# JSzitas/nlsolver

Hardware: AMD Instinct MI355X
Metric: candidate-evals/sec (pop x iters/s) Rosenbrock-128D DE (higher is better)
Workload: dtype f64; 1 GPU; Rosenbrock-128D DE strategy=random CR=0.9 F=0.8, pop=65536 per GPU (BASELINE configs[1]), one step = best scan + std_err + stop tests + one generation; global_pop=65536, dim=128

## Files before the change

nlsolver_amd/csrc/nlsg_common.h:

```cpp
#pragma once

#ifdef __HIPCC_RTC__
typedef unsigned long long uint64_t;
typedef long long int64_t;
typedef unsigned int uint32_t;
typedef int int32_t;
typedef unsigned char uint8_t;
#else
#include <hip/hip_runtime.h>
#include <stdint.h>

#include <atomic>
#include <chrono>
#include <cstdarg>
#include <cstdio>
#include <cstring>
#endif

#include "../../include/nlsg_c_api.h"
#include "nlsg_math.h"
#ifndef __HIPCC_RTC__
#include "nlsg_pool.h"
#endif

// ... 137 lines not shown
  const uint32_t hi = lane_xor32<OFF>(static_cast<uint32_t>(v >> 32));
  return (static_cast<uint64_t>(hi) << 32) | lo;
}
template <int OFF>
__device__ inline double lane_xor(double v) {
  return __longlong_as_double(static_cast<long long>(
      lane_xor<OFF>(static_cast<uint64_t>(__double_as_longlong(v)))));
}
__device__ inline double lane_down1(double v) {
  const uint64_t b = static_cast<uint64_t>(__double_as_longlong(v));
  const uint32_t lo = dpp_mov32<0x130, 0xF>(static_cast<uint32_t>(b), static_cast<uint32_t>(b));
  const uint32_t hi = dpp_mov32<0x130, 0xF>(static_cast<uint32_t>(b >> 32), static_cast<uint32_t>(b >> 32));
  return __longlong_as_double(static_cast<long long>((static_cast<uint64_t>(hi) << 32) | lo));
}
__device__ inline double lane_up1(double v) {
  const uint64_t b = static_cast<uint64_t>(__double_as_longlong(v));
  const uint32_t lo = dpp_mov32<0x138, 0xF>(static_cast<uint32_t>(b), static_cast<uint32_t>(b));
  const uint32_t hi = dpp_mov32<0x138, 0xF>(static_cast<uint32_t>(b >> 32), static_cast<uint32_t>(b >> 32));
  return __longlong_as_double(static_cast<long long>((static_cast<uint64_t>(hi) << 32) | lo));
}
__device__ inline double lane_first(double v) {
  const uint64_t b = static_cast<uint64_t>(__double_as_longlong(v));
  const uint32_t lo = __builtin_amdgcn_readfirstlane(static_cast<int>(b & 0xffffffffu));
  const uint32_t hi = __builtin_amdgcn_readfirstlane(static_cast<int>(b >> 32));
  return __longlong_as_double(static_cast<long long>((static_cast<uint64_t>(hi) << 32) | lo));
}
__device__ inline double lane_last(double v) {
  const uint64_t b = static_cast<uint64_t>(__double_as_longlong(v));
  const uint32_t lo = __builtin_amdgcn_readlane(static_cast<int>(b & 0xffffffffu), 63);
  const uint32_t hi = __builtin_amdgcn_readlane(static_cast<int>(b >> 32), 63);
  return __longlong_as_double(static_cast<long long>((static_cast<uint64_t>(hi) << 32) | lo));
}
__device__ inline uint64_t on_valu(uint64_t s) {
  const uint32_t lo = static_cast<uint32_t>(s), hi = static_cast<uint32_t>(s >> 32);
  uint32_t vlo, vhi;
  asm("v_mov_b32 %0, %1" : "=v"(vlo) : "s"(lo));
  asm("v_mov_b32 %0, %1" : "=v"(vhi) : "s"(hi));
  return (static_cast<uint64_t>(vhi) << 32) | vlo;
}
__device__ inline uint64_t first64(uint64_t v) {
  const uint32_t lo = __builtin_amdgcn_readfirstlane(static_cast<int>(v & 0xffffffffu));
  const uint32_t hi = __builtin_amdgcn_readfirstlane(static_cast<int>(v >> 32));
  return (static_cast<uint64_t>(hi) << 32) | lo;
}
__device__ inline uint64_t readlane64(uint64_t v, int src) {
  const uint32_t lo = __builtin_amdgcn_readlane(static_cast<int>(v & 0xffffffffu), src);
  const uint32_t hi = __builtin_amdgcn_readlane(static_cast<int>(v >> 32), src);
  return (static_cast<uint64_t>(hi) << 32) | lo;
}
__device__ inline double lane_broadcast(double v, int src) {
  return __longlong_as_double(static_cast<long long>(
      readlane64(static_cast<uint64_t>(__double_as_longlong(v)), src)));
}
__device__ inline bool lane_bit(uint64_t m) {
#if __has_builtin(__builtin_amdgcn_inverse_ballot_w64)
  return __builtin_amdgcn_inverse_ballot_w64(m);
#else
  uint32_t r;
  asm("v_cndmask_b32_e64 %0, 0, 1, %1" : "=v"(r) : "s"(m));
  return r != 0;
#endif
}
template <int N>
struct int_c {
  static constexpr int value = N;
};
template <int FIRST, typename F>
__device__ inline void butterfly_levels(F &&f) {
  f(int_c<FIRST>{});
  if constexpr (FIRST > 1) butterfly_levels<FIRST / 2>(f);
}

template <int CTRL, int BANK>
__device__ inline uint32_t dpp_fresh32(uint32_t src) {
  return static_cast<uint32_t>(__builtin_amdgcn_mov_dpp(static_cast<int>(src), CTRL, 0xF, BANK, true));
}
template <int OFF>
__device__ inline double xor_add(double v) {
  static_assert(OFF == 1 || OFF == 2 || OFF == 4 || OFF == 8 || OFF == 16 || OFF == 32, "");
  const uint64_t b = static_cast<uint64_t>(__double_as_longlong(v));
  const uint32_t lo = static_cast<uint32_t>(b), hi = static_cast<uint32_t>(b >> 32);
  auto f64 = [](uint32_t l, uint32_t h) {
    return __longlong_as_double(static_cast<long long>((static_cast<uint64_t>(h) << 32) | l));
  };
  if constexpr (OFF == 16 || OFF == 32) {
    if constexpr (OFF == 16) {
      const auto rl = __builtin_amdgcn_permlane16_swap(lo, lo, false, false);
      const auto rh = __builtin_amdgcn_permlane16_swap(hi, hi, false, false);
      return f64(rl[0], rh[0]) + f64(rl[1], rh[1]);
    } else {
      const auto rl = __builtin_amdgcn_permlane32_swap(lo, lo, false, false);
      const auto rh = __builtin_amdgcn_permlane32_swap(hi, hi, false, false);
      return f64(rl[0], rh[0]) + f64(rl[1], rh[1]);
    }
  } else if constexpr (OFF == 4) {
    const uint32_t pl = dpp_mov32<0x114, 0xA>(dpp_fresh32<0x104, 0x5>(lo), lo);
    const uint32_t ph = dpp_mov32<0x114, 0xA>(dpp_fresh32<0x104, 0x5>(hi), hi);
    return v + f64(pl, ph);
  } else {
    constexpr int ctrl = OFF == 1 ? 0xB1 : OFF == 2 ? 0x4E : 0x128;
    return v + f64(dpp_fresh32<ctrl, 0xF>(lo), dpp_fresh32<ctrl, 0xF>(hi));
  }
}

__device__ inline double wave_sum(double v) {
  butterfly_levels<32>([&](auto off) { v = xor_add<decltype(off)::value>(v); });
// ... 640 lines not shown
```

nlsolver_amd/csrc/nlsg_de_kernels.h:

```cpp
#pragma once

#include "nlsg_common.h"
#include "nlsg_de_state.h"

namespace nlsg {

constexpr int kTraceWords = 5;

struct DeParams {
  double *buf[2];
  double *scores[2];
  uint8_t *home[2];
  double *best_x;
  uint64_t *trace;
  DeState *state;
  TilePartial *part;
  uint32_t *ticket;
  const double *zero;
  uint32_t ntiles;
  uint32_t stream;
  uint64_t pop, D, shard_lo, shard_n;
  double CR, F, eps, fmul;
  uint64_t max_iter, best_val_no_change, seed;
  int32_t strategy;
// ... 332 lines not shown
  const uint32_t d32 = static_cast<uint32_t>(D);
  auto row = [&](uint32_t h, uint64_t local) {
    return ((h & 1u) ? p.buf[1] : p.buf[0]) + static_cast<uint64_t>(static_cast<uint32_t>(local)) * d32;
  };
  auto load2 = [&](const double *rp, double (&v)[2]) {
    v[0] = in0 ? rp[j0] : 0.0;
    v[1] = in1 ? rp[j1] : 0.0;
  };
  double d1[2], d2[2], d3[2], keep[2];
  load2(row(hp[r0 - p.shard_lo], r0 - p.shard_lo), d1);
  load2(row(hp[r1 - p.shard_lo], r1 - p.shard_lo), d2);
  load2(row(hp[r2 - p.shard_lo], r2 - p.shard_lo), d3);
  const double *ks = rnd ? row(ha, a) : p.best_x;
  keep[0] = (in0 && !cross[0]) ? ks[j0] : 0.0;
  keep[1] = (in1 && !cross[1]) ? ks[j1] : 0.0;
  const double old_score = p.scores[par][a];
  double trial[2];
#pragma unroll
  for (int k = 0; k < 2; k++) {
    const double mut = d1[k] + p.F * (d2[k] - d3[k]);
    const double t = cross[k] ? mut : keep[k];
    trial[k] = (k ? in1 : in0) ? t : 0.0;
  }
  const double score = p.fmul * group_objective<OBJ, G>(trial[0], trial[1], D);
  const bool accept = score < old_score;
  if (live) {
    if (accept) {
      double *out = row(ha ^ 1u, a);
      if (in0) out[j0] = trial[0];
      if (in1) out[j1] = trial[1];
    }
    if (g == 0) {
      p.scores[par ^ 1][a] = accept ? score : old_score;
      p.home[par ^ 1][a] = static_cast<uint8_t>(accept ? ha ^ 1u : ha);
      if (p.trace != nullptr) {
        uint64_t *t = p.trace + a * kTraceWords;
        t[0] = r0;
        t[1] = r1;
        t[2] = r2;
        t[3] = jrand;
        t[4] = accept ? 1u : 0u;
      }
    }
  }
}

template <int OBJ, int G>
__global__ __launch_bounds__(256) void de_generation_groups_kernel(DeParams p, int par,
                                                                   uint64_t generation,
                                                                   int ignore_done) {
  de_generation_groups_block<OBJ, G>(p, par, generation, ignore_done, blockIdx.x);
}

template <int OBJ, bool VEC>
__device__ inline void de_generation_pair(const DeParams &p, int par, uint64_t generation, uint64_t block) {
  static_assert(TermsNonNegative<OBJ>::value, "the screen needs terms >= 0");
  using O = Objective<OBJ>;
  const uint64_t a0 = 2 * (block * 4 + __builtin_amdgcn_readfirstlane(static_cast<int>(threadIdx.x) >> 6));
  if (a0 >= p.shard_n) return;
  const bool two = a0 + 1 < p.shard_n;
  const int lane = lane_id();
  const uint32_t j = static_cast<uint32_t>(lane) & 31u;
  const bool upper = lane >= 32;
  const bool live = !upper || two;
  const uint32_t a = static_cast<uint32_t>(a0) + ((upper && two) ? 1u : 0u);
  const uint8_t *__restrict__ hp = p.home[par];
  const uint32_t hraw = hp[a];
  double old_score = p.scores[par][a];
  const uint32_t d32 = static_cast<uint32_t>(p.D);
  const uint64_t ka = ctr_key(p.gen_key, p.shard_lo + a);
  const uint32_t lim = j == 0 ? d32 : static_cast<uint32_t>(p.shard_n);
  const uint32_t idx = static_cast<uint32_t>(u01(mix64(ka + golden_times(d32 + j + 1u))) * static_cast<double>(lim));
  const uint32_t drawn = idx >= lim ? lim - 1 : idx;
  uint32_t sel = hraw;
  asm("" : "+v"(sel), "+v"(old_score) : "v"(drawn));
  const uint32_t cnt = (sel >> 2) & 3u;
  const bool tries = live & de_screen_tries(sel, generation, a, p.retry_mask, p.screen_retry_mask);
  bool dec = false;
  uint32_t left = cnt << 2;
  if (__ballot(tries) != 0ull) {
    const uint32_t hsel = hp[(j >= 1 && j < 8) ? drawn : a];
    auto half_of = [&](uint32_t lo, uint32_t hi) { return upper ? hi : lo; };
    auto lane32 = [&](uint32_t v, int src) {
      return static_cast<uint32_t>(__builtin_amdgcn_readlane(static_cast<int>(v), src));
    };
    const uint32_t jrand = half_of(lane32(drawn, 0), lane32(drawn, 32));
    constexpr uint32_t top = 1u << 31;
    const uint64_t b0 = __ballot(drawn != a) & ~0x0000000100000001ull;
    const uint32_t m0l = static_cast<uint32_t>(b0), m0h = static_cast<uint32_t>(b0 >> 32);
    const int i0l = __builtin_ctz(m0l | top), i0h = __builtin_ctz(m0h | top);
    const uint32_t r0 = half_of(lane32(drawn, i0l), lane32(drawn, 32 + i0h));
    const uint64_t b1 = __ballot(drawn != r0);
    const uint32_t m1l = m0l & static_cast<uint32_t>(b1) & ((~0u << i0l) << 1);
    const uint32_t m1h = m0h & static_cast<uint32_t>(b1 >> 32) & ((~0u << i0h) << 1);
    const int i1l = __builtin_ctz(m1l | top), i1h = __builtin_ctz(m1h | top);
    const uint32_t r1 = half_of(lane32(drawn, i1l), lane32(drawn, 32 + i1h));
    const uint64_t b2 = __ballot(drawn != r1);
    const uint32_t m2l = m1l & static_cast<uint32_t>(b2) & ((~0u << i1l) << 1);
    const uint32_t m2h = m1h & static_cast<uint32_t>(b2 >> 32) & ((~0u << i1h) << 1);
    const int i2l = __builtin_ctz(m2l | top), i2h = __builtin_ctz(m2h | top);
    const uint32_t r2 = half_of(lane32(drawn, i2l), lane32(drawn, 32 + i2h));
    const bool okl = m0l != 0 && m1l != 0 && m2l != 0 && i2l < 8;
    const bool okh = m0h != 0 && m1h != 0 && m2h != 0 && i2h < 8;
    const bool run = tries && (upper ? okh : okl);
    const uint32_t h0 = half_of(lane32(hsel, i0l), lane32(hsel, 32 + i0h));
    const uint32_t h1 = half_of(lane32(hsel, i1l), lane32(hsel, 32 + i1h));
    const uint32_t h2 = half_of(lane32(hsel, i2l), lane32(hsel, 32 + i2h));
    const uint64_t ka_lane = ka + golden_times(2 * j + 1u);
    const bool c0 = mix64(ka_lane) < p.cr_thresh || p.cr_all || 2 * j == jrand;
    const bool c1 = mix64(ka_lane + kGolden) < p.cr_thresh || p.cr_all || 2 * j + 1 == jrand;
    typedef double __attribute__((address_space(1))) global_double;
    global_double *base0 = (global_double *)p.buf[0], *base1 = (global_double *)p.buf[1];
    asm("" : "+s"(base0), "+s"(base1));
    auto load2 = [&](uint32_t h, uint32_t r, double (&v)[2]) {
      const double *src = (double *)((h & 1u) ? base1 : base0) + static_cast<uint64_t>(r) * d32 + 2 * j;
      if (VEC) {
        const double2 t = *reinterpret_cast<const double2 *>(src);
        v[0] = t.x;
        v[1] = t.y;
      } else {
        v[0] = src[0];
        v[1] = src[1];
      }
    };
    double d1[2], d2[2], d3[2];
    load2(h0, r0, d1);
    load2(h1, r1, d2);
    load2(h2, r2, d3);
    const double x0 = d1[0] + p.F * (d2[0] - d3[0]);
    const double x1 = d1[1] + p.F * (d2[1] - d3[1]);
    const double xn = lane_down1(x0);
    const bool cn = lane_bit(__ballot(c0) >> 1) && j != 31;
    const bool k0 = c0 && (O::kChain ? c1 : true);
    const bool k1 = c1 && (O::kChain ? cn : j != 31);
    double acc = 0.0;
    acc = acc + (k0 ? O::term(x0, x1) : 0.0);
    acc = acc + (k1 ? O::term(x1, xn) : 0.0);
    butterfly_levels<16>([&](auto off) { acc = xor_add<decltype(off)::value>(acc); });
    dec = run && acc >= old_score;
    left = de_screen_count_after(cnt, dec ? 0 : run ? 1 : 2) << 2;
    if (j == 0 && dec) {
      p.scores[par ^ 1][a] = old_score;
      p.home[par ^ 1][a] = static_cast<uint8_t>(hraw & 1u);
      if (p.trace != nullptr) {
        uint64_t *t = p.trace + static_cast<uint64_t>(a) * kTraceWords;
        t[0] = p.shard_lo + r0;
        t[1] = p.shard_lo + r1;
        t[2] = p.shard_lo + r2;
        t[3] = jrand;
        t[4] = 0u;
      }
    }
    if (p.counts != nullptr && j == 0 && run) {
      if (dec) atomicAdd(reinterpret_cast<unsigned long long *>(p.counts + kDeBoundDecided), 1ull);
      atomicAdd(reinterpret_cast<unsigned long long *>(p.counts + (dec ? kDeScreenDecided : kDeScreenMissed)), 1ull);
    }
  }
  const uint64_t decided = __ballot(dec);
  if (((a0 >> 1) & 63u) == 0) {
    asm volatile("" ::: "memory");
    if (decided != 0ull && lane == 0)
      atomicAdd(p.ticket + kDeScreenStat, static_cast<uint32_t>(__builtin_popcountll(decided & 0x0000000100000001ull)));
  }
  if ((~decided & (two ? 0x0000000100000001ull : 1ull)) == 0ull) return;
  const uint32_t left_l = static_cast<uint32_t>(__builtin_amdgcn_readlane(static_cast<int>(left), 0));
  const uint32_t left_h = static_cast<uint32_t>(__builtin_amdgcn_readlane(static_cast<int>(left), 32));
  const uint64_t best_id = p.state->best_id;
  auto one_agent = [&](int h) {
    DeAgent<1> A;
    de_fetch_agent<true, 1, VEC>(p, par, p.gen_key, generation, best_id, a0 + h, A);
    A.miss = h ? left_h : left_l;
    de_process_agent<OBJ, 1, VEC, true>(p, par, A);
  };
  if (!(decided & 1ull)) one_agent(0);
  if (two && !((decided >> 32) & 1ull)) one_agent(1);
}

template <int OBJ, int CHUNKS, bool VEC, bool BOUND = false, bool SCREEN = false>
__device__ inline void de_generation_block(const DeParams &p, int par, uint64_t generation,
                                           int ignore_done, uint64_t block) {
  const DeState *__restrict__ st = p.state;
  if (!ignore_done && st->done) return;
  if constexpr (SCREEN) {
    static_assert(BOUND && CHUNKS == 1, "the screen rides on the bound, rows of 65..128 coordinates");
    de_generation_pair<OBJ, VEC>(p, par, generation, block);
    return;
  }
  const uint64_t a0 = block * 4 + __builtin_amdgcn_readfirstlane(static_cast<int>(threadIdx.x) >> 6);
  if (a0 >= p.shard_n) return;
  const uint64_t kg = p.gen_key;
  const uint64_t best_id = st->best_id;
  DeAgent<CHUNKS> A;
  de_fetch_agent<BOUND, CHUNKS, VEC>(p, par, kg, generation, best_id, a0, A);
  de_process_agent<OBJ, CHUNKS, VEC, BOUND>(p, par, A);
}

template <int OBJ, int CHUNKS, bool VEC, bool BOUND = false, bool SCREEN = false>
__global__ __launch_bounds__(256) void de_generation_kernel(DeParams p, int par, uint64_t generation,
                                                          int ignore_done) {
  de_generation_block<OBJ, CHUNKS, VEC, BOUND, SCREEN>(p, par, generation, ignore_done, blockIdx.x);
}

__global__ __launch_bounds__(256) void de_gather_kernel(DeParams p, int par, double *__restrict__ out) {
  for (uint64_t r = blockIdx.x; r < p.shard_n; r += gridDim.x) {
    const double *__restrict__ src = de_row(p, p.home[par][r], r);
    for (uint64_t d = threadIdx.x; d < p.D; d += 256) out[r * p.D + d] = src[d];
  }
}

__device__ inline bool take_ticket(const DeParams &p) { return take_ticket(p.ticket, p.ntiles); }

__device__ inline void de_scan_head_block(const DeParams &p, uint64_t k, uint32_t tile, double *rec) {
  __shared__ double red[4];
  __shared__ double mv[4];
  __shared__ uint64_t mi[4];
  __shared__ uint64_t s_row;
  __shared__ int s_have;
  __shared__ int s_last;
  DeState *st = p.state;
  if (st->done) return;
  const int par = static_cast<int>(k & 1);
  const bool need_se = p.eps > 0;
  const double *__restrict__ sc = p.scores[par];
  const uint64_t base = static_cast<uint64_t>(tile) * kTile;
  const uint64_t tile_n = (p.shard_n - base) < kTile ? (p.shard_n - base) : kTile;
  double v[kTile / 256];
  double acc = 0.0;
  double bv = __builtin_inf();
  uint64_t bi = ~0ull;
#pragma unroll
  for (int q = 0; q < kTile / 256; q++) {
    const uint64_t i = threadIdx.x + 256u * q;
    v[q] = sc[base + (i < tile_n ? i : 0)];
  }
#pragma unroll
  for (int q = 0; q < kTile / 256; q++) {
    const uint64_t i = threadIdx.x + 256u * q;
    if (i < tile_n) {
      acc = acc + v[q];
      argmin_combine(bv, bi, v[q], base + i);
    }
  }
  double tile_sum = 0.0, tile_m2 = 0.0;
  if (need_se) {
    tile_sum = block_tree_256(acc, red);
    const double tile_mean = tile_sum / static_cast<double>(tile_n);
    acc = 0.0;
#pragma unroll
    for (int q = 0; q < kTile / 256; q++) {
      const double d = v[q] - tile_mean;
      if (threadIdx.x + 256u * q < tile_n) acc = acc + d * d;
// ... 26 lines not shown
    total = block_tree_256(acc, red);
    const double mean = total / static_cast<double>(p.shard_n);
    acc = 0.0;
    for (uint32_t j = threadIdx.x; j < p.ntiles; j += 256) {
      const uint64_t jb = static_cast<uint64_t>(j) * kTile;
      const double nj = static_cast<double>((p.shard_n - jb) < kTile ? (p.shard_n - jb) : kTile);
      const double mj = sc1_load(&p.part[j].sum) / nj;
      const double dm = mj == mean ? 0.0 : mj - mean;
      acc = acc + (sc1_load(&p.part[j].m2) + nj * (dm * dm));
    }
    m2 = block_tree_256(acc, red);
  }
  if (threadIdx.x == 0) {
    const uint64_t inc = st->best_id;
    uint64_t gi = (bi == ~0ull) ? inc : p.shard_lo + bi;
    if (inc >= p.shard_lo && inc < p.shard_lo + p.shard_n) {
      const double inc_score = sc[inc - p.shard_lo];
      if (!(bv < inc_score)) {
        gi = inc;
        bv = inc_score;
      }
    }
    const bool mine = gi >= p.shard_lo && gi < p.shard_lo + p.shard_n;
    if (rec == nullptr) {
      finish_turn(st, p, gi, bv, mine,
                  need_se ? sqrt(m2 / static_cast<double>(p.pop - 1))
                          : __builtin_nan(""));
    } else {
      rec[0] = bv;
      rec[1] = __longlong_as_double(static_cast<long long>(gi));
      rec[2] = total;
      rec[3] = m2;
      rec[4] = mine ? 1.0 : 0.0;
    }
    s_row = gi - p.shard_lo;
    s_have = mine ? 1 : 0;
  }
  __syncthreads();
  const bool have = s_have != 0;
  const uint64_t r = have ? s_row : 0;
  const double *row = de_row(p, p.home[par][r], r);
  if (rec != nullptr) {
    for (uint64_t d = threadIdx.x; d < p.D; d += 256) rec[kRecHeader + d] = have ? row[d] : 0.0;
  } else if (have) {
    for (uint64_t d = threadIdx.x; d < p.D; d += 256) p.best_x[d] = row[d];
  }
}

__global__ __launch_bounds__(256) void de_scan_head_kernel(DeParams p, uint64_t k, double *rec) {
  de_scan_head_block(p, k, blockIdx.x, rec);
}

template <int OBJ, int CHUNKS, bool VEC, bool BOUND = false, bool SCREEN = false>
__global__ __launch_bounds__(256) void de_turn_kernel(DeParams p, int par, uint64_t generation) {
  if (blockIdx.x < p.ntiles) {
    de_scan_head_block(p, generation - 1, blockIdx.x, nullptr);
    return;
  }
  de_generation_block<OBJ, CHUNKS, VEC, BOUND, SCREEN>(p, par, generation, 0, blockIdx.x - p.ntiles);
}

template <int OBJ, int G>
__global__ __launch_bounds__(256) void de_turn_groups_kernel(DeParams p, int par, uint64_t generation) {
  if (blockIdx.x < p.ntiles) {
    de_scan_head_block(p, generation - 1, blockIdx.x, nullptr);
    return;
  }
  de_generation_groups_block<OBJ, G>(p, par, generation, 0, blockIdx.x - p.ntiles);
}

__global__ __launch_bounds__(256) void de_finalize_kernel(DeParams p, const double *recs,
                                                        int32_t world, uint64_t rec_stride) {
  __shared__ int s_win;
  DeState *st = p.state;
  if (st->done) return;
  if (threadIdx.x == 0) {
    const uint64_t inc = st->best_id;
    int win = -1;
    double bv = __builtin_inf();
    uint64_t bi = inc;
    for (int r = 0; r < world; r++) {
      const double *rec = recs + static_cast<uint64_t>(r) * rec_stride;
      if (rec[4] != 1.0) continue;
      const double v = rec[0];
      const uint64_t i = static_cast<uint64_t>(__double_as_longlong(rec[1]));
      if (i == inc && v != v) {
        bv = v;
        bi = i;
        win = r;
        break;
      }
      const bool better =
          win < 0 || v < bv || (v == bv && bi != inc && (i == inc || i < bi));
      if (better) {
        bv = v;
        bi = i;
        win = r;
      }
    }
    double se = __builtin_nan("");
    if (p.eps > 0) {
      const double n_r = static_cast<double>(p.shard_n);
      double tot = 0.0;
      for (int r = 0; r < world; r++) tot = tot + recs[static_cast<uint64_t>(r) * rec_stride + 2];
      const double gmean = tot / static_cast<double>(p.pop);
      double m2 = 0.0;
      for (int r = 0; r < world; r++) {
// ... 148 lines not shown
```

nlsolver_amd/csrc/nlsg_de_state.h:

```cpp
#pragma once

#ifndef __HIPCC_RTC__
#include <cstdlib>
#endif

#include "nlsg_common.h"

namespace nlsg {

constexpr int kDeMaxTries = 64;

struct DeState {
  uint64_t best_id;
  double best_f;
  uint64_t iter;
  uint64_t val_no_change;
  uint64_t fcalls;
  double std_err;
  int32_t done;
  int32_t parity;
  int32_t pad[2];
};

template <typename P>
// ... 14 lines not shown
  if (st->iter >= p.max_iter || st->val_no_change >= p.best_val_no_change ||
      (p.eps > 0 && se < p.eps)) {
    st->done = 1;
  }
}

template <typename P>
inline void set_crossover_test(P &p, double cr) {
  p.cr_all = 0;
  if (u01(~0ull) < cr) {
    p.cr_all = 1;
    p.cr_thresh = ~0ull;
  } else if (!(u01(0) < cr)) {
    p.cr_thresh = 0;
  } else {
    uint64_t lo = 0, hi = ~0ull;
    while (hi - lo > 1) {
      const uint64_t mid = lo + (hi - lo) / 2;
      if (u01(mid) < cr) lo = mid; else hi = mid;
    }
    p.cr_thresh = hi;
  }
}

#ifndef __HIPCC_RTC__
constexpr double kDeBoundMinCR = 0.8, kDeBoundMaxCR = 1.0;
constexpr uint32_t kDeBoundRetry = 256;
inline bool de_bound_gate(int objective, int strategy, bool minimize, double cr, uint64_t dim,
                          double min_cr = kDeBoundMinCR, double max_cr = kDeBoundMaxCR) {
  return (objective == NLSG_OBJ_ROSENBROCK || objective == NLSG_OBJ_SPHERE) &&
         strategy == NLSG_DE_RANDOM && minimize && dim >= 65 && dim <= 1024 && cr >= min_cr &&
         cr < max_cr;
}

constexpr uint32_t kDeScreenRetry = 16;
inline bool de_screen_gate(int objective, int strategy, bool minimize, double cr, uint64_t dim,
                           double min_cr = kDeBoundMinCR, double max_cr = kDeBoundMaxCR) {
  return de_bound_gate(objective, strategy, minimize, cr, dim, min_cr, max_cr) && dim >= 65 && dim <= 128;
}
inline void de_screen_env(const char *screen, const char *retry, bool *on, uint32_t *period) {
  *on = !(screen && screen[0] == '0');
  *period = kDeScreenRetry;
  if (retry) {
    const long r = std::atol(retry);
    if (r >= 1 && r <= (1l << 30) && (r & (r - 1)) == 0) *period = static_cast<uint32_t>(r);
  }
}

#endif

__host__ __device__ inline bool de_screen_tries(uint32_t sel, uint64_t generation, uint32_t a,
                                                uint32_t bound_retry_mask, uint32_t screen_retry_mask) {
  const uint32_t ga = static_cast<uint32_t>(generation) + a;
  const bool bound_tries = ((sel & 2u) == 0) | ((ga & bound_retry_mask) == 0);
  const uint32_t cnt = (sel >> 2) & 3u;
  return bound_tries & ((cnt < 2) | ((ga & screen_retry_mask) == 0));
}
__host__ __device__ inline uint32_t de_screen_count_after(uint32_t cnt, int outcome) {
  return outcome == 0 ? 0u : outcome == 1 ? (cnt < 3 ? cnt + 1 : 3u) : cnt;
}

}
```

nlsolver_amd/csrc/nlsg_de.hip:

```cpp
#include <algorithm>
#include <cmath>
#include <cstdlib>

#include "nlsg_comm.h"
#include "nlsg_de_kernels.h"
#include "nlsg_engine.h"
#include "nlsg_rtc.h"

using namespace nlsg;

struct nlsg_de : EngineBase {
  nlsg_de_config cfg;
  DeParams p;
  double *x0_dev = nullptr;
  double *zero_dev = nullptr;
  double *rec = nullptr;
  int chunks = 0;
  int group = 0;
  bool long_rows = false;
  bool initialised = false;
  uint64_t k = 0;
  hipStream_t side = nullptr;
  hipEvent_t ev_gen[4] = {nullptr, nullptr, nullptr, nullptr};
  hipEvent_t ev_head[4] = {nullptr, nullptr, nullptr, nullptr};
// ... 46 lines not shown

void launch_init(nlsg_de *e) {
  const dim3 grid(static_cast<unsigned>((e->p.shard_n + 3) / 4)), block(256);
  if (e->cfg.objective == NLSG_OBJ_CUSTOM) {
    void *args[] = {&e->p, &e->x0_dev};
    launch_module(e, e->rtc.init, grid.x, args);
    return;
  }
  if (e->long_rows) {
#define CALL(OBJ)                                                                              \
  if (e->p.vec)                                                                                \
    hipLaunchKernelGGL((de_init_long_kernel<OBJ, true>), grid, block, 0, e->stream, e->p, e->x0_dev); \
  else                                                                                         \
    hipLaunchKernelGGL((de_init_long_kernel<OBJ, false>), grid, block, 0, e->stream, e->p, e->x0_dev)
    NLSG_FOR_OBJ_LONG(e->cfg.objective, CALL)
#undef CALL
    return;
  }
#define CALL(OBJ, C)                                                                          \
  if (e->p.vec)                                                                               \
    hipLaunchKernelGGL((de_init_kernel<OBJ, C, true>), grid, block, 0, e->stream, e->p,       \
                       e->x0_dev);                                                            \
  else                                                                                        \
    hipLaunchKernelGGL((de_init_kernel<OBJ, C, false>), grid, block, 0, e->stream, e->p,      \
                       e->x0_dev)
  NLSG_FOR_OBJ(e->cfg.objective, e->chunks, CALL)
#undef CALL
}

template <int OBJ>
void launch_generation_groups(nlsg_de *e, dim3 grid, int par, uint64_t generation, int ignore_done) {
  const dim3 block(256);
  switch (e->group) {
    case 4:
      hipLaunchKernelGGL((de_generation_groups_kernel<OBJ, 4>), grid, block, 0, e->stream, e->p, par,
                         generation, ignore_done);
      break;
    case 8:
      hipLaunchKernelGGL((de_generation_groups_kernel<OBJ, 8>), grid, block, 0, e->stream, e->p, par,
                         generation, ignore_done);
      break;
    case 16:
      hipLaunchKernelGGL((de_generation_groups_kernel<OBJ, 16>), grid, block, 0, e->stream, e->p, par,
                         generation, ignore_done);
      break;
    default:
      hipLaunchKernelGGL((de_generation_groups_kernel<OBJ, 32>), grid, block, 0, e->stream, e->p, par,
                         generation, ignore_done);
      break;
  }
}

uint64_t generation_waves(const nlsg_de *e) {
  const uint64_t per_wave = (e->p.bound & kDeBoundScreen) ? 2 : e->group ? 64 / e->group : 1;
  return (e->p.shard_n + per_wave - 1) / per_wave;
}

void launch_generation(nlsg_de *e, int par, uint64_t generation, int ignore_done = 0) {
  e->p.gen_key = ctr_key(e->p.seed, generation);
  const uint64_t waves = generation_waves(e);
  const dim3 grid(static_cast<unsigned>((waves + 3) / 4)), block(256);
  if (e->cfg.objective == NLSG_OBJ_CUSTOM) {
    void *args[] = {&e->p, &par, &generation, &ignore_done};
    launch_module(e, e->rtc.generation, grid.x, args);
    return;
  }
  if (e->long_rows) {
#define CALL(OBJ)                                                                               \
  if (e->p.vec)                                                                                 \
    hipLaunchKernelGGL((de_generation_long_kernel<OBJ, true>), grid, block, 0, e->stream, e->p, \
                       par, generation, ignore_done);                                           \
  else                                                                                          \
    hipLaunchKernelGGL((de_generation_long_kernel<OBJ, false>), grid, block, 0, e->stream, e->p, \
                       par, generation, ignore_done)
    NLSG_FOR_OBJ_LONG(e->cfg.objective, CALL)
#undef CALL
    return;
  }
  if (e->group) {
    switch (e->cfg.objective) {
      case NLSG_OBJ_ROSENBROCK:
        launch_generation_groups<NLSG_OBJ_ROSENBROCK>(e, grid, par, generation, ignore_done);
        break;
      case NLSG_OBJ_SPHERE:
        launch_generation_groups<NLSG_OBJ_SPHERE>(e, grid, par, generation, ignore_done);
        break;
      case NLSG_OBJ_STYBLINSKI_TANG:
        launch_generation_groups<NLSG_OBJ_STYBLINSKI_TANG>(e, grid, par, generation, ignore_done);
        break;
      default:
        launch_generation_groups<NLSG_OBJ_RASTRIGIN>(e, grid, par, generation, ignore_done);
        break;
    }
    return;
  }
#define CALL_B(OBJ, C, V, B, S)                                                                   \
  hipLaunchKernelGGL((de_generation_kernel<OBJ, C, V, B, S>), grid, block, 0, e->stream, e->p, par, \
                     generation, ignore_done)
#define CALL(OBJ, C)                                                          \
  if (e->p.bound & kDeBoundScreen) {                                          \
    if (e->p.vec) CALL_B(OBJ, C, true, TermsNonNegative<OBJ>::value, (TermsNonNegative<OBJ>::value && C == 1));  \
    else CALL_B(OBJ, C, false, TermsNonNegative<OBJ>::value, (TermsNonNegative<OBJ>::value && C == 1));          \
  } else if (e->p.bound) {                                                    \
    if (e->p.vec) CALL_B(OBJ, C, true, TermsNonNegative<OBJ>::value, false);  \
    else CALL_B(OBJ, C, false, TermsNonNegative<OBJ>::value, false);          \
  } else if (e->p.vec) CALL_B(OBJ, C, true, false, false);                    \
  else CALL_B(OBJ, C, false, false, false)
// ... 659 lines not shown
```

Before: 3.362 billion candidate-evals/s.

## Add fast path for distinct donor selection via DPP and bpermute in DE pair kernel

In the paired-agent DE generation path, a fast path checks with two DPP row shifts and ballots whether the first drawn lanes already give distinct donors. When they do, it gathers jrand, donors and home bits with ds_bpermute per half instead of the serial chain of readlanes, ctz and ballots, which stays as a fallback. Screen-tries and decision logic become wave-uniform scalar values read from lanes 0 and 32, so the per-lane count bookkeeping and one ballot are dropped. The fast path brings LDS-permute latency and extra ballots, and the donor choice must still match the fallback.

New measurement: 3.312 billion candidate-evals/s. 0.985x the previous value.

```diff
diff --git a/nlsolver_amd/csrc/nlsg_common.h b/nlsolver_amd/csrc/nlsg_common.h
--- a/nlsolver_amd/csrc/nlsg_common.h
+++ b/nlsolver_amd/csrc/nlsg_common.h
@@ -213,6 +213,19 @@
   return __longlong_as_double(static_cast<long long>(
       readlane64(static_cast<uint64_t>(__double_as_longlong(v)), src)));
 }
+__device__ inline uint32_t half_index() { return (static_cast<uint32_t>(threadIdx.x) & 32u) << 2; }
+template <int K>
+__device__ inline uint32_t half_lane(uint32_t v, uint32_t index) {
+  static_assert(K >= 0 && K < 32, "a lane of the own half");
+  return static_cast<uint32_t>(
+      __builtin_amdgcn_ds_bpermute(static_cast<int>(index + 4u * K), static_cast<int>(v)));
+}
+template <int N>
+__device__ inline uint32_t row_down(uint32_t v) {
+  static_assert(N == 1 || N == 2, "");
+  return static_cast<uint32_t>(__builtin_amdgcn_mov_dpp(static_cast<int>(v), 0x100 + N, 0xF, 0xF, true));
+}
+
 __device__ inline bool lane_bit(uint64_t m) {
 #if __has_builtin(__builtin_amdgcn_inverse_ballot_w64)
   return __builtin_amdgcn_inverse_ballot_w64(m);
diff --git a/nlsolver_amd/csrc/nlsg_de_kernels.h b/nlsolver_amd/csrc/nlsg_de_kernels.h
--- a/nlsolver_amd/csrc/nlsg_de_kernels.h
+++ b/nlsolver_amd/csrc/nlsg_de_kernels.h
@@ -414,54 +414,79 @@
   using O = Objective<OBJ>;
   const uint64_t a0 = 2 * (block * 4 + __builtin_amdgcn_readfirstlane(static_cast<int>(threadIdx.x) >> 6));
   if (a0 >= p.shard_n) return;
-  const bool two = a0 + 1 < p.shard_n;
+  const bool two = static_cast<uint32_t>(a0) + 1u < static_cast<uint32_t>(p.shard_n);
   const int lane = lane_id();
   const uint32_t j = static_cast<uint32_t>(lane) & 31u;
   const bool upper = lane >= 32;
-  const bool live = !upper || two;
   const uint32_t a = static_cast<uint32_t>(a0) + ((upper && two) ? 1u : 0u);
   const uint8_t *__restrict__ hp = p.home[par];
   const uint32_t hraw = hp[a];
   double old_score = p.scores[par][a];
   const uint32_t d32 = static_cast<uint32_t>(p.D);
-  const uint64_t ka = ctr_key(p.gen_key, p.shard_lo + a);
+  const uint64_t ga0 = p.shard_lo + a0;
+  const uint64_t ka_lo = ctr_key(p.gen_key, ga0), ka_hi = ctr_key(p.gen_key, ga0 + 1);
+  const uint64_t ka = upper ? ka_hi : ka_lo;
   const uint32_t lim = j == 0 ? d32 : static_cast<uint32_t>(p.shard_n);
   const uint32_t idx = static_cast<uint32_t>(u01(mix64(ka + golden_times(d32 + j + 1u))) * static_cast<double>(lim));
   const uint32_t drawn = idx >= lim ? lim - 1 : idx;
   uint32_t sel = hraw;
   asm("" : "+v"(sel), "+v"(old_score) : "v"(drawn));
-  const uint32_t cnt = (sel >> 2) & 3u;
-  const bool tries = live & de_screen_tries(sel, generation, a, p.retry_mask, p.screen_retry_mask);
-  bool dec = false;
-  uint32_t left = cnt << 2;
-  if (__ballot(tries) != 0ull) {
-    const uint32_t hsel = hp[(j >= 1 && j < 8) ? drawn : a];
-    auto half_of = [&](uint32_t lo, uint32_t hi) { return upper ? hi : lo; };
-    auto lane32 = [&](uint32_t v, int src) {
-      return static_cast<uint32_t>(__builtin_amdgcn_readlane(static_cast<int>(v), src));
-    };
-    const uint32_t jrand = half_of(lane32(drawn, 0), lane32(drawn, 32));
-    constexpr uint32_t top = 1u << 31;
-    const uint64_t b0 = __ballot(drawn != a) & ~0x0000000100000001ull;
-    const uint32_t m0l = static_cast<uint32_t>(b0), m0h = static_cast<uint32_t>(b0 >> 32);
-    const int i0l = __builtin_ctz(m0l | top), i0h = __builtin_ctz(m0h | top);
-    const uint32_t r0 = half_of(lane32(drawn, i0l), lane32(drawn, 32 + i0h));
-    const uint64_t b1 = __ballot(drawn != r0);
-    const uint32_t m1l = m0l & static_cast<uint32_t>(b1) & ((~0u << i0l) << 1);
-    const uint32_t m1h = m0h & static_cast<uint32_t>(b1 >> 32) & ((~0u << i0h) << 1);
-    const int i1l = __builtin_ctz(m1l | top), i1h = __builtin_ctz(m1h | top);
-    const uint32_t r1 = half_of(lane32(drawn, i1l), lane32(drawn, 32 + i1h));
-    const uint64_t b2 = __ballot(drawn != r1);
-    const uint32_t m2l = m1l & static_cast<uint32_t>(b2) & ((~0u << i1l) << 1);
-    const uint32_t m2h = m1h & static_cast<uint32_t>(b2 >> 32) & ((~0u << i1h) << 1);
-    const int i2l = __builtin_ctz(m2l | top), i2h = __builtin_ctz(m2h | top);
-    const uint32_t r2 = half_of(lane32(drawn, i2l), lane32(drawn, 32 + i2h));
-    const bool okl = m0l != 0 && m1l != 0 && m2l != 0 && i2l < 8;
-    const bool okh = m0h != 0 && m1h != 0 && m2h != 0 && i2h < 8;
-    const bool run = tries && (upper ? okh : okl);
-    const uint32_t h0 = half_of(lane32(hsel, i0l), lane32(hsel, 32 + i0h));
-    const uint32_t h1 = half_of(lane32(hsel, i1l), lane32(hsel, 32 + i1h));
-    const uint32_t h2 = half_of(lane32(hsel, i2l), lane32(hsel, 32 + i2h));
+  const uint32_t sel_lo = static_cast<uint32_t>(__builtin_amdgcn_readlane(static_cast<int>(sel), 0));
+  const uint32_t sel_hi = static_cast<uint32_t>(__builtin_amdgcn_readlane(static_cast<int>(sel), 32));
+  const uint32_t al = static_cast<uint32_t>(a0);
+  const bool tries_lo = de_screen_tries(sel_lo, generation, al, p.retry_mask, p.screen_retry_mask);
+  const bool tries_hi = two && de_screen_tries(sel_hi, generation, al + 1u, p.retry_mask, p.screen_retry_mask);
+  constexpr uint64_t kLower = 0x00000000ffffffffull, kFirst = 0x0000000100000001ull;
+  bool run_lo = false, run_hi = false;
+  uint64_t dec_m = 0;
+  if (tries_lo || tries_hi) {
+    const uint32_t hsel = hp[(j >= 1 && j < 8) ? drawn : a] & 1u;
+    const uint64_t b0 = __ballot(drawn != a) & ~kFirst;
+    const uint64_t n1 = __ballot(drawn != row_down<1>(drawn));
+    const uint64_t n2 = __ballot(drawn != row_down<2>(drawn));
+    const uint64_t b01 = b0 & n1;
+    const uint64_t plain = b01 & (b01 >> 1) & (b0 >> 2) & n2;
+    uint32_t jrand, r0, r1, r2, h0, h1, h2;
+    bool ok_lo, ok_hi;
+    if (__builtin_expect((~plain & (two ? kFirst << 1 : 2ull)) == 0ull, 1)) {
+      const uint32_t hi = half_index();
+      jrand = half_lane<0>(drawn, hi);
+      r0 = half_lane<1>(drawn, hi);
+      r1 = half_lane<2>(drawn, hi);
+      r2 = half_lane<3>(drawn, hi);
+      h0 = half_lane<1>(hsel, hi);
+      h1 = half_lane<2>(hsel, hi);
+      h2 = half_lane<3>(hsel, hi);
+      ok_lo = ok_hi = true;
+    } else {
+      auto half_of = [&](uint32_t lo, uint32_t hi) { return upper ? hi : lo; };
+      auto lane32 = [&](uint32_t v, int src) {
+        return static_cast<uint32_t>(__builtin_amdgcn_readlane(static_cast<int>(v), src));
+      };
+      jrand = half_of(lane32(drawn, 0), lane32(drawn, 32));
+      constexpr uint32_t top = 1u << 31;
+      const uint32_t m0l = static_cast<uint32_t>(b0), m0h = static_cast<uint32_t>(b0 >> 32);
+      const int i0l = __builtin_ctz(m0l | top), i0h = __builtin_ctz(m0h | top);
+      r0 = half_of(lane32(drawn, i0l), lane32(drawn, 32 + i0h));
+      const uint64_t b1 = __ballot(drawn != r0);
+      const uint32_t m1l = m0l & static_cast<uint32_t>(b1) & ((~0u << i0l) << 1);
+      const uint32_t m1h = m0h & static_cast<uint32_t>(b1 >> 32) & ((~0u << i0h) << 1);
+      const int i1l = __builtin_ctz(m1l | top), i1h = __builtin_ctz(m1h | top);
+      r1 = half_of(lane32(drawn, i1l), lane32(drawn, 32 + i1h));
+      const uint64_t b2 = __ballot(drawn != r1);
+      const uint32_t m2l = m1l & static_cast<uint32_t>(b2) & ((~0u << i1l) << 1);
+      const uint32_t m2h = m1h & static_cast<uint32_t>(b2 >> 32) & ((~0u << i1h) << 1);
+      const int i2l = __builtin_ctz(m2l | top), i2h = __builtin_ctz(m2h | top);
+      r2 = half_of(lane32(drawn, i2l), lane32(drawn, 32 + i2h));
+      ok_lo = m0l != 0 && m1l != 0 && m2l != 0 && i2l < 8;
+      ok_hi = m0h != 0 && m1h != 0 && m2h != 0 && i2h < 8;
+      h0 = half_of(lane32(hsel, i0l), lane32(hsel, 32 + i0h));
+      h1 = half_of(lane32(hsel, i1l), lane32(hsel, 32 + i1h));
+      h2 = half_of(lane32(hsel, i2l), lane32(hsel, 32 + i2h));
+    }
+    run_lo = tries_lo && ok_lo;
+    run_hi = tries_hi && ok_hi;
+    const uint64_t run_m = (run_lo ? kLower : 0ull) | (run_hi ? ~kLower : 0ull);
     const uint64_t ka_lane = ka + golden_times(2 * j + 1u);
     const bool c0 = mix64(ka_lane) < p.cr_thresh || p.cr_all || 2 * j == jrand;
     const bool c1 = mix64(ka_lane + kGolden) < p.cr_thresh || p.cr_all || 2 * j + 1 == jrand;
@@ -469,7 +494,7 @@
     global_double *base0 = (global_double *)p.buf[0], *base1 = (global_double *)p.buf[1];
     asm("" : "+s"(base0), "+s"(base1));
     auto load2 = [&](uint32_t h, uint32_t r, double (&v)[2]) {
-      const double *src = (double *)((h & 1u) ? base1 : base0) + static_cast<uint64_t>(r) * d32 + 2 * j;
+      const double *src = (double *)(h ? base1 : base0) + static_cast<uint64_t>(r) * d32 + 2 * j;
       if (VEC) {
         const double2 t = *reinterpret_cast<const double2 *>(src);
         v[0] = t.x;
@@ -493,8 +518,8 @@
     acc = acc + (k0 ? O::term(x0, x1) : 0.0);
     acc = acc + (k1 ? O::term(x1, xn) : 0.0);
     butterfly_levels<16>([&](auto off) { acc = xor_add<decltype(off)::value>(acc); });
-    dec = run && acc >= old_score;
-    left = de_screen_count_after(cnt, dec ? 0 : run ? 1 : 2) << 2;
+    dec_m = __ballot(acc >= old_score) & run_m;
+    const bool dec = lane_bit(dec_m);
     if (j == 0 && dec) {
       p.scores[par ^ 1][a] = old_score;
       p.home[par ^ 1][a] = static_cast<uint8_t>(hraw & 1u);
@@ -507,20 +532,23 @@
         t[4] = 0u;
       }
     }
-    if (p.counts != nullptr && j == 0 && run) {
+    if (p.counts != nullptr && j == 0 && lane_bit(run_m)) {
       if (dec) atomicAdd(reinterpret_cast<unsigned long long *>(p.counts + kDeBoundDecided), 1ull);
       atomicAdd(reinterpret_cast<unsigned long long *>(p.counts + (dec ? kDeScreenDecided : kDeScreenMissed)), 1ull);
     }
   }
-  const uint64_t decided = __ballot(dec);
+  const uint64_t decided = dec_m;
   if (((a0 >> 1) & 63u) == 0) {
     asm volatile("" ::: "memory");
     if (decided != 0ull && lane == 0)
-      atomicAdd(p.ticket + kDeScreenStat, static_cast<uint32_t>(__builtin_popcountll(decided & 0x0000000100000001ull)));
-  }
-  if ((~decided & (two ? 0x0000000100000001ull : 1ull)) == 0ull) return;
-  const uint32_t left_l = static_cast<uint32_t>(__builtin_amdgcn_readlane(static_cast<int>(left), 0));
-  const uint32_t left_h = static_cast<uint32_t>(__builtin_amdgcn_readlane(static_cast<int>(left), 32));
+      atomicAdd(p.ticket + kDeScreenStat, static_cast<uint32_t>(__builtin_popcountll(decided & kFirst)));
+  }
+  if ((~decided & (two ? kFirst : 1ull)) == 0ull) return;
+  auto left_of = [&](uint32_t s, bool d, bool run) {
+    return de_screen_count_after((s >> 2) & 3u, d ? 0 : run ? 1 : 2) << 2;
+  };
+  const uint32_t left_l = left_of(sel_lo, decided & 1ull, run_lo);
+  const uint32_t left_h = left_of(sel_hi, (decided >> 32) & 1ull, run_hi);
   const uint64_t best_id = p.state->best_id;
   auto one_agent = [&](int h) {
     DeAgent<1> A;
diff --git a/nlsolver_amd/csrc/nlsg_de_state.h b/nlsolver_amd/csrc/nlsg_de_state.h
--- a/nlsolver_amd/csrc/nlsg_de_state.h
+++ b/nlsolver_amd/csrc/nlsg_de_state.h
@@ -90,9 +90,9 @@
 __host__ __device__ inline bool de_screen_tries(uint32_t sel, uint64_t generation, uint32_t a,
                                                 uint32_t bound_retry_mask, uint32_t screen_retry_mask) {
   const uint32_t ga = static_cast<uint32_t>(generation) + a;
-  const bool bound_tries = ((sel & 2u) == 0) | ((ga & bound_retry_mask) == 0);
+  const bool bound_tries = (sel & 2u) == 0 || (ga & bound_retry_mask) == 0;
   const uint32_t cnt = (sel >> 2) & 3u;
-  return bound_tries & ((cnt < 2) | ((ga & screen_retry_mask) == 0));
+  return bound_tries && (cnt < 2 || (ga & screen_retry_mask) == 0);
 }
 __host__ __device__ inline uint32_t de_screen_count_after(uint32_t cnt, int outcome) {
   return outcome == 0 ? 0u : outcome == 1 ? (cnt < 3 ? cnt + 1 : 3u) : cnt;
```

## Screen four agents per wave with LDS plans and software-pipelined row loads

Applied to the files above, without the earlier changes.

The DE screening kernel now handles four agents per wavefront in two passes instead of two agents in one pass. Index drawing and duplicate rejection are done with eight-lane groups using DPP compares and ballots. Each group writes a small per-agent plan of row pointers, score, key and jrand into LDS, and the pass loop prefetches the next pass's donor rows while evaluating the current one. Waves-per-EU hints are also raised for the screen kernels to push occupancy. In exchange the code adds LDS traffic, a wave barrier and register pressure, and generation_waves is adjusted to match the new agents per wave.

Result: faster. 3.370 billion candidate-evals/s before, 3.583 billion candidate-evals/s after (median of 6 runs) (+6.3%).

```diff
diff --git a/nlsolver_amd/csrc/nlsg_de.hip b/nlsolver_amd/csrc/nlsg_de.hip
--- a/nlsolver_amd/csrc/nlsg_de.hip
+++ b/nlsolver_amd/csrc/nlsg_de.hip
@@ -122,7 +122,7 @@
 }
 
 uint64_t generation_waves(const nlsg_de *e) {
-  const uint64_t per_wave = (e->p.bound & kDeBoundScreen) ? 2 : e->group ? 64 / e->group : 1;
+  const uint64_t per_wave = (e->p.bound & kDeBoundScreen) ? kDeScreenAgents : e->group ? 64 / e->group : 1;
   return (e->p.shard_n + per_wave - 1) / per_wave;
 }
 
diff --git a/nlsolver_amd/csrc/nlsg_de_kernels.h b/nlsolver_amd/csrc/nlsg_de_kernels.h
--- a/nlsolver_amd/csrc/nlsg_de_kernels.h
+++ b/nlsolver_amd/csrc/nlsg_de_kernels.h
@@ -408,70 +408,93 @@
   de_generation_groups_block<OBJ, G>(p, par, generation, ignore_done, blockIdx.x);
 }
 
-template <int OBJ, bool VEC>
-__device__ inline void de_generation_pair(const DeParams &p, int par, uint64_t generation, uint64_t block) {
+constexpr int kDeScreenPasses = 2;
+constexpr int kDeScreenAgents = 2 * kDeScreenPasses;
+constexpr int kDePlanWords = 16;
+
+template <int OBJ, bool VEC, int NP = kDeScreenPasses>
+__device__ inline void de_generation_screen(const DeParams &p, int par, uint64_t generation, uint64_t block) {
   static_assert(TermsNonNegative<OBJ>::value, "the screen needs terms >= 0");
   using O = Objective<OBJ>;
-  const uint64_t a0 = 2 * (block * 4 + __builtin_amdgcn_readfirstlane(static_cast<int>(threadIdx.x) >> 6));
+  typedef double __attribute__((address_space(1))) global_double;
+  typedef double __attribute__((ext_vector_type(2))) double_x2;
+  typedef double_x2 __attribute__((address_space(1))) global_double_x2;
+  __shared__ __attribute__((aligned(16))) uint32_t plans[4 * 8 * kDePlanWords];
+  const uint32_t tid = threadIdx.x;
+  constexpr uint32_t per_wave = 2 * NP;
+  const uint64_t a0 = per_wave * (block * 4 + __builtin_amdgcn_readfirstlane(static_cast<int>(tid >> 6)));
   if (a0 >= p.shard_n) return;
-  const bool two = a0 + 1 < p.shard_n;
-  const int lane = lane_id();
-  const uint32_t j = static_cast<uint32_t>(lane) & 31u;
+  const uint64_t rest = p.shard_n - a0;
+  const uint32_t n_live = rest < per_wave ? static_cast<uint32_t>(rest) : per_wave;
+  const uint32_t lane = tid & 63u;
+  const uint32_t d32 = static_cast<uint32_t>(p.D);
+  global_double *base0 = (global_double *)p.buf[0], *base1 = (global_double *)p.buf[1];
+  asm("" : "+s"(base0), "+s"(base1));
+  {
+    const uint32_t c = lane & 7u, q = lane >> 3;
+    const bool live = q < n_live;
+    const uint32_t a = static_cast<uint32_t>(a0) + (live ? q : 0u);
+    const uint8_t *__restrict__ hp = p.home[par];
+    const uint64_t ka = ctr_key(p.gen_key, p.shard_lo + a);
+    const uint32_t lim = c == 0 ? d32 : static_cast<uint32_t>(p.shard_n);
+    const uint32_t idx = static_cast<uint32_t>(u01(mix64(ka + golden_times(d32 + c + 1u))) * static_cast<double>(lim));
+    const uint32_t drawn = idx >= lim ? lim - 1 : idx;
+    const uint32_t sel = hp[c == 0 ? a : drawn];
+    const double old_score = p.scores[par][a];
+    constexpr uint64_t each = 0x0101010101010101ull;
+    uint64_t dup = __ballot(dpp_mov32<0x111, 0xF>(drawn, drawn) == drawn) & (0xFCull * each);
+    dup |= __ballot(dpp_mov32<0x112, 0xF>(drawn, drawn) == drawn) & (0xF8ull * each);
+    dup |= __ballot(dpp_mov32<0x113, 0xF>(drawn, drawn) == drawn) & (0xF0ull * each);
+    dup |= __ballot(dpp_mov32<0x114, 0xF>(drawn, drawn) == drawn) & (0xE0ull * each);
+    dup |= __ballot(dpp_mov32<0x115, 0xF>(drawn, drawn) == drawn) & (0xC0ull * each);
+    dup |= __ballot(dpp_mov32<0x116, 0xF>(drawn, drawn) == drawn) & (0x80ull * each);
+    const uint64_t keep = __ballot(drawn != a) & ~dup & (0xFEull * each);
+    const uint32_t grp = static_cast<uint32_t>(keep >> (lane & 56u)) & 0xFFu;
+    const uint32_t rank = static_cast<uint32_t>(__builtin_popcount(grp & ((1u << c) - 1u)));
+    const bool ok = __builtin_popcount(grp) >= 3;
+    const bool mine = ((grp >> c) & 1u) != 0 && rank < 3;
+    const bool run = live & ok & de_screen_tries(sel, generation, a, p.retry_mask, p.screen_retry_mask);
+    uint32_t *rec = plans + (tid >> 3) * kDePlanWords;
+    if (c == 0) {
+      const uint64_t b = reinterpret_cast<uint64_t>(base0);
+      const uint64_t os = static_cast<uint64_t>(__double_as_longlong(old_score));
+      const uint32_t bl = static_cast<uint32_t>(b), bh = static_cast<uint32_t>(b >> 32);
+      *reinterpret_cast<uint4 *>(rec) = make_uint4(bl, bh, bl, bh);
+      *reinterpret_cast<uint4 *>(rec + 4) =
+          make_uint4(bl, bh, static_cast<uint32_t>(ka), static_cast<uint32_t>(ka >> 32));
+      *reinterpret_cast<uint4 *>(rec + 8) = make_uint4(static_cast<uint32_t>(os), static_cast<uint32_t>(os >> 32),
+                                                       drawn, (sel & 0xFFu) | (run ? 0x100u : 0u));
+    }
+    if (mine) {
+      global_double *row = ((sel & 1u) ? base1 : base0) + static_cast<uint64_t>(drawn) * d32;
+      *reinterpret_cast<uint64_t *>(rec + 2 * rank) = reinterpret_cast<uint64_t>(row);
+      rec[12 + rank] = drawn;
+    }
+  }
+  __builtin_amdgcn_fence(__ATOMIC_RELEASE, "wavefront");
+  __builtin_amdgcn_wave_barrier();
+  __builtin_amdgcn_fence(__ATOMIC_ACQUIRE, "wavefront");
+  const uint32_t j = lane & 31u;
   const bool upper = lane >= 32;
-  const bool live = !upper || two;
-  const uint32_t a = static_cast<uint32_t>(a0) + ((upper && two) ? 1u : 0u);
-  const uint8_t *__restrict__ hp = p.home[par];
-  const uint32_t hraw = hp[a];
-  double old_score = p.scores[par][a];
-  const uint32_t d32 = static_cast<uint32_t>(p.D);
-  const uint64_t ka = ctr_key(p.gen_key, p.shard_lo + a);
-  const uint32_t lim = j == 0 ? d32 : static_cast<uint32_t>(p.shard_n);
-  const uint32_t idx = static_cast<uint32_t>(u01(mix64(ka + golden_times(d32 + j + 1u))) * static_cast<double>(lim));
-  const uint32_t drawn = idx >= lim ? lim - 1 : idx;
-  uint32_t sel = hraw;
-  asm("" : "+v"(sel), "+v"(old_score) : "v"(drawn));
-  const uint32_t cnt = (sel >> 2) & 3u;
-  const bool tries = live & de_screen_tries(sel, generation, a, p.retry_mask, p.screen_retry_mask);
-  bool dec = false;
-  uint32_t left = cnt << 2;
-  if (__ballot(tries) != 0ull) {
-    const uint32_t hsel = hp[(j >= 1 && j < 8) ? drawn : a];
-    auto half_of = [&](uint32_t lo, uint32_t hi) { return upper ? hi : lo; };
-    auto lane32 = [&](uint32_t v, int src) {
-      return static_cast<uint32_t>(__builtin_amdgcn_readlane(static_cast<int>(v), src));
-    };
-    const uint32_t jrand = half_of(lane32(drawn, 0), lane32(drawn, 32));
-    constexpr uint32_t top = 1u << 31;
-    const uint64_t b0 = __ballot(drawn != a) & ~0x0000000100000001ull;
-    const uint32_t m0l = static_cast<uint32_t>(b0), m0h = static_cast<uint32_t>(b0 >> 32);
-    const int i0l = __builtin_ctz(m0l | top), i0h = __builtin_ctz(m0h | top);
-    const uint32_t r0 = half_of(lane32(drawn, i0l), lane32(drawn, 32 + i0h));
-    const uint64_t b1 = __ballot(drawn != r0);
-    const uint32_t m1l = m0l & static_cast<uint32_t>(b1) & ((~0u << i0l) << 1);
-    const uint32_t m1h = m0h & static_cast<uint32_t>(b1 >> 32) & ((~0u << i0h) << 1);
-    const int i1l = __builtin_ctz(m1l | top), i1h = __builtin_ctz(m1h | top);
-    const uint32_t r1 = half_of(lane32(drawn, i1l), lane32(drawn, 32 + i1h));
-    const uint64_t b2 = __ballot(drawn != r1);
-    const uint32_t m2l = m1l & static_cast<uint32_t>(b2) & ((~0u << i1l) << 1);
-    const uint32_t m2h = m1h & static_cast<uint32_t>(b2 >> 32) & ((~0u << i1h) << 1);
-    const int i2l = __builtin_ctz(m2l | top), i2h = __builtin_ctz(m2h | top);
-    const uint32_t r2 = half_of(lane32(drawn, i2l), lane32(drawn, 32 + i2h));
-    const bool okl = m0l != 0 && m1l != 0 && m2l != 0 && i2l < 8;
-    const bool okh = m0h != 0 && m1h != 0 && m2h != 0 && i2h < 8;
-    const bool run = tries && (upper ? okh : okl);
-    const uint32_t h0 = half_of(lane32(hsel, i0l), lane32(hsel, 32 + i0h));
-    const uint32_t h1 = half_of(lane32(hsel, i1l), lane32(hsel, 32 + i1h));
-    const uint32_t h2 = half_of(lane32(hsel, i2l), lane32(hsel, 32 + i2h));
-    const uint64_t ka_lane = ka + golden_times(2 * j + 1u);
-    const bool c0 = mix64(ka_lane) < p.cr_thresh || p.cr_all || 2 * j == jrand;
-    const bool c1 = mix64(ka_lane + kGolden) < p.cr_thresh || p.cr_all || 2 * j + 1 == jrand;
-    typedef double __attribute__((address_space(1))) global_double;
-    global_double *base0 = (global_double *)p.buf[0], *base1 = (global_double *)p.buf[1];
-    asm("" : "+s"(base0), "+s"(base1));
-    auto load2 = [&](uint32_t h, uint32_t r, double (&v)[2]) {
-      const double *src = (double *)((h & 1u) ? base1 : base0) + static_cast<uint64_t>(r) * d32 + 2 * j;
+  const uint32_t *plan0 = plans + (tid >> 6) * (8 * kDePlanWords) + (upper ? kDePlanWords : 0);
+  struct Pass {
+    double old_score;
+    uint32_t jrand, flags;
+    double d1[2], d2[2], d3[2];
+  };
+  auto fetch = [&](int i, Pass &R) {
+    const uint32_t *rd = plan0 + i * (2 * kDePlanWords);
+    const uint4 w0 = *reinterpret_cast<const uint4 *>(rd);
+    const uint2 w1 = *reinterpret_cast<const uint2 *>(rd + 4);
+    const uint4 w2 = *reinterpret_cast<const uint4 *>(rd + 8);
+    auto u64 = [](uint32_t lo, uint32_t hi) { return (static_cast<uint64_t>(hi) << 32) | lo; };
+    R.old_score = __longlong_as_double(static_cast<long long>(u64(w2.x, w2.y)));
+    R.jrand = w2.z;
+    R.flags = w2.w;
+    auto load2 = [&](uint64_t row, double (&v)[2]) {
+      const global_double *src = reinterpret_cast<const global_double *>(row) + 2 * j;
       if (VEC) {
-        const double2 t = *reinterpret_cast<const double2 *>(src);
+        const double_x2 t = *reinterpret_cast<const global_double_x2 *>(src);
         v[0] = t.x;
         v[1] = t.y;
       } else {
@@ -479,31 +502,46 @@
         v[1] = src[1];
       }
     };
-    double d1[2], d2[2], d3[2];
-    load2(h0, r0, d1);
-    load2(h1, r1, d2);
-    load2(h2, r2, d3);
-    const double x0 = d1[0] + p.F * (d2[0] - d3[0]);
-    const double x1 = d1[1] + p.F * (d2[1] - d3[1]);
+    load2(u64(w0.x, w0.y), R.d1);
+    load2(u64(w0.z, w0.w), R.d2);
+    load2(u64(w1.x, w1.y), R.d3);
+  };
+  const uint64_t golden_j = golden_times(2 * j + 1u);
+  const uint64_t cr_all = p.cr_all ? ~0ull : 0ull;
+  uint64_t known0[NP], known1[NP];
+  auto masks = [&](int i) {
+    const uint32_t *rd = plan0 + i * (2 * kDePlanWords);
+    const uint64_t ka_lane = *reinterpret_cast<const uint64_t *>(rd + 6) + golden_j;
+    const uint32_t jrand = rd[10];
+    const uint64_t c0 = __ballot(mix64(ka_lane) < p.cr_thresh) | cr_all | __ballot(2 * j == jrand);
+    const uint64_t c1 = __ballot(mix64(ka_lane + kGolden) < p.cr_thresh) | cr_all | __ballot(2 * j + 1 == jrand);
+    constexpr uint64_t not31 = ~((1ull << 31) | (1ull << 63));
+    known0[i] = O::kChain ? (c0 & c1) : c0;
+    known1[i] = c1 & (O::kChain ? (c0 >> 1) : ~0ull) & not31;
+  };
+  uint32_t decided = 0;
+  uint32_t lefts = 0;
+  auto rows = [&](int i, const Pass &R, double x0, double x1) {
+    const uint32_t a = static_cast<uint32_t>(a0) + 2 * i + (upper ? 1u : 0u);
+    const bool run = (R.flags & 0x100u) != 0;
+    const uint32_t cnt = (R.flags >> 2) & 3u;
     const double xn = lane_down1(x0);
-    const bool cn = lane_bit(__ballot(c0) >> 1) && j != 31;
-    const bool k0 = c0 && (O::kChain ? c1 : true);
-    const bool k1 = c1 && (O::kChain ? cn : j != 31);
     double acc = 0.0;
-    acc = acc + (k0 ? O::term(x0, x1) : 0.0);
-    acc = acc + (k1 ? O::term(x1, xn) : 0.0);
+    acc = acc + (lane_bit(known0[i]) ? O::term(x0, x1) : 0.0);
+    acc = acc + (lane_bit(known1[i]) ? O::term(x1, xn) : 0.0);
     butterfly_levels<16>([&](auto off) { acc = xor_add<decltype(off)::value>(acc); });
-    dec = run && acc >= old_score;
-    left = de_screen_count_after(cnt, dec ? 0 : run ? 1 : 2) << 2;
+    const bool dec = run && acc >= R.old_score;
+    lefts |= (de_screen_count_after(cnt, dec ? 0 : run ? 1 : 2) << 2) << (8 * i);
     if (j == 0 && dec) {
-      p.scores[par ^ 1][a] = old_score;
-      p.home[par ^ 1][a] = static_cast<uint8_t>(hraw & 1u);
+      p.scores[par ^ 1][a] = R.old_score;
+      p.home[par ^ 1][a] = static_cast<uint8_t>(R.flags & 1u);
       if (p.trace != nullptr) {
+        const uint32_t *rd = plan0 + i * (2 * kDePlanWords);
         uint64_t *t = p.trace + static_cast<uint64_t>(a) * kTraceWords;
-        t[0] = p.shard_lo + r0;
-        t[1] = p.shard_lo + r1;
-        t[2] = p.shard_lo + r2;
-        t[3] = jrand;
+        t[0] = p.shard_lo + rd[12];
+        t[1] = p.shard_lo + rd[13];
+        t[2] = p.shard_lo + rd[14];
+        t[3] = R.jrand;
         t[4] = 0u;
       }
     }
@@ -511,25 +549,41 @@
       if (dec) atomicAdd(reinterpret_cast<unsigned long long *>(p.counts + kDeBoundDecided), 1ull);
       atomicAdd(reinterpret_cast<unsigned long long *>(p.counts + (dec ? kDeScreenDecided : kDeScreenMissed)), 1ull);
     }
-  }
-  const uint64_t decided = __ballot(dec);
-  if (((a0 >> 1) & 63u) == 0) {
-    asm volatile("" ::: "memory");
-    if (decided != 0ull && lane == 0)
-      atomicAdd(p.ticket + kDeScreenStat, static_cast<uint32_t>(__builtin_popcountll(decided & 0x0000000100000001ull)));
-  }
-  if ((~decided & (two ? 0x0000000100000001ull : 1ull)) == 0ull) return;
-  const uint32_t left_l = static_cast<uint32_t>(__builtin_amdgcn_readlane(static_cast<int>(left), 0));
-  const uint32_t left_h = static_cast<uint32_t>(__builtin_amdgcn_readlane(static_cast<int>(left), 32));
+    const uint64_t d = __ballot(dec);
+    decided |= ((static_cast<uint32_t>(d) & 1u) | ((static_cast<uint32_t>(d >> 32) & 1u) << 1)) << (2 * i);
+    if (i == 0 && (a0 & 127u) == 0) {
+      asm volatile("" ::: "memory");
+      if (d != 0ull && lane == 0)
+        atomicAdd(p.ticket + kDeScreenStat, static_cast<uint32_t>(__builtin_popcountll(d & 0x0000000100000001ull)));
+    }
+  };
+  Pass R[2];
+  fetch(0, R[0]);
+  if (NP > 1) fetch(1, R[1]);
+#pragma unroll
+  for (int i = 0; i < NP; i++) masks(i);
+#pragma unroll
+  for (int i = 0; i < NP; i++) {
+    Pass &C = R[i & 1];
+    const Pass S = C;
+    const double x0 = C.d1[0] + p.F * (C.d2[0] - C.d3[0]);
+    const double x1 = C.d1[1] + p.F * (C.d2[1] - C.d3[1]);
+    if (i + 2 < NP) fetch(i + 2, C);
+    rows(i, S, x0, x1);
+  }
+  uint32_t undecided = ~decided & ((1u << n_live) - 1u);
+  if (undecided == 0) return;
+  const uint32_t lefts_l = static_cast<uint32_t>(__builtin_amdgcn_readlane(static_cast<int>(lefts), 0));
+  const uint32_t lefts_h = static_cast<uint32_t>(__builtin_amdgcn_readlane(static_cast<int>(lefts), 32));
   const uint64_t best_id = p.state->best_id;
-  auto one_agent = [&](int h) {
+  do {
+    const uint32_t q = static_cast<uint32_t>(__builtin_ctz(undecided));
+    undecided &= undecided - 1u;
     DeAgent<1> A;
-    de_fetch_agent<true, 1, VEC>(p, par, p.gen_key, generation, best_id, a0 + h, A);
-    A.miss = h ? left_h : left_l;
+    de_fetch_agent<true, 1, VEC>(p, par, p.gen_key, generation, best_id, a0 + q, A);
+    A.miss = (((q & 1u) ? lefts_h : lefts_l) >> (8 * (q >> 1))) & 0xCu;
     de_process_agent<OBJ, 1, VEC, true>(p, par, A);
-  };
-  if (!(decided & 1ull)) one_agent(0);
-  if (two && !((decided >> 32) & 1ull)) one_agent(1);
+  } while (undecided != 0);
 }
 
 template <int OBJ, int CHUNKS, bool VEC, bool BOUND = false, bool SCREEN = false>
@@ -539,7 +593,7 @@
   if (!ignore_done && st->done) return;
   if constexpr (SCREEN) {
     static_assert(BOUND && CHUNKS == 1, "the screen rides on the bound, rows of 65..128 coordinates");
-    de_generation_pair<OBJ, VEC>(p, par, generation, block);
+    de_generation_screen<OBJ, VEC>(p, par, generation, block);
     return;
   }
   const uint64_t a0 = block * 4 + __builtin_amdgcn_readfirstlane(static_cast<int>(threadIdx.x) >> 6);
@@ -552,7 +606,7 @@
 }
 
 template <int OBJ, int CHUNKS, bool VEC, bool BOUND = false, bool SCREEN = false>
-__global__ __launch_bounds__(256) void de_generation_kernel(DeParams p, int par, uint64_t generation,
+__global__ __launch_bounds__(256) __attribute__((amdgpu_waves_per_eu(SCREEN ? 8 : 1, 8))) void de_generation_kernel(DeParams p, int par, uint64_t generation,
                                                           int ignore_done) {
   de_generation_block<OBJ, CHUNKS, VEC, BOUND, SCREEN>(p, par, generation, ignore_done, blockIdx.x);
 }
@@ -685,7 +739,7 @@
 }
 
 template <int OBJ, int CHUNKS, bool VEC, bool BOUND = false, bool SCREEN = false>
-__global__ __launch_bounds__(256) void de_turn_kernel(DeParams p, int par, uint64_t generation) {
+__global__ __launch_bounds__(256) __attribute__((amdgpu_waves_per_eu(SCREEN ? 8 : 1, 8))) void de_turn_kernel(DeParams p, int par, uint64_t generation) {
   if (blockIdx.x < p.ntiles) {
     de_scan_head_block(p, generation - 1, blockIdx.x, nullptr);
     return;
```
